# kcat/openal-soft

Measured on AMD Instinct MI355X. Metric: mixed voices/sec @48kHz 1024-sample update, HRTF stereo; fraction of HBM roofline, higher is better.
Workload: dtype f32

## Files before the change

### openal-soft_amd/csrc/api.hip

```cpp
#include "api_context.hpp"
namespace oalgpu {

thread_local std::string gLastError;

int Fail(int code, const std::string &msg)
{
    gLastError = msg;
    return code;
}

void ParkResidentContexts(int device);

int UseDevice(int device)
{
    int count = 0;
    if(hipGetDeviceCount(&count) != hipSuccess || count <= 0)
        return Fail(OALGPU_ERR_NO_DEVICE, "no HIP device available (the product has no CPU path)");
    if(device < 0 || device >= count) return Fail(OALGPU_ERR_INVALID, "device ordinal out of range");
    HIP_TRY(hipSetDevice(device));
    ParkResidentContexts(device);
    return OALGPU_OK;
}

}
// ... 493 lines not shown
        else (void)hipGetLastError();
    }
    return ResidentGiveUp(c, std::string(e < 4 ? what[e] : "a wait timed out") + state);
}

static int ResidentSubmit(oalgpu_context *c, uint32_t samples_to_do)
{
    auto &R = c->res;
    if(!R.ready) { if(int rc = ResidentInit(c)) return R.failed ? 1 : rc; }
    HIP_TRY(hipSetDevice(c->desc.device));
    using clk = std::chrono::steady_clock;
    std::unique_lock<std::mutex> g(gResLock);
    const DeviceLayout &L = c->L;
    const bool launchNow = !R.running;
    ResidentArgs a{};
    uint32_t evk = 0;
    bool timed = false;
    if(launchNow)
    {
        if(c->postPending) HIP_TRY(hipStreamWaitEvent(R.reduceStream, c->lastPostEvent ? c->lastPostEvent : c->evPostDone, 0));
        const uint32_t k = evk = R.launches % oalgpu_context::ResidentState::kEv;
        if(R.evOpen[k]) { HIP_TRY(hipEventSynchronize(R.evStop[k])); ResidentCollectTimes(c, false); }
        timed = R.timeLaunches;
        a.door = R.door; a.counters = R.counters.p; a.hostFlags = R.hostFlags; a.partBase = R.part.p; a.setStride = uint32_t(R.setFloats);
        a.base = R.next; a.endSeq = R.next + R.maxUpdates; a.redPerUpdate = R.redGroups;
        a.startedTarget = R.startedTotal + L.numGroups; a.launchId = R.launches + 1u;
        __atomic_store_n(&R.door->exitSeq[a.launchId & 3u], R.next + 0x40000000u, __ATOMIC_RELEASE);
        __atomic_store_n(&R.door->seq, R.next, __ATOMIC_RELEASE);
        __builtin_ia32_sfence();
    }
    {
        const auto deadline = clk::now() + std::chrono::seconds(5);
        uint32_t spins = 0;
        while(int32_t(R.posts - __atomic_load_n(R.hostFlags + 16u * kRhProgress, __ATOMIC_ACQUIRE)) >= int32_t(kResidentDepth))
        {
            __builtin_ia32_pause();
            if((++spins & 0x3ffu) == 0 && clk::now() > deadline)
            {
                ResidentParkLocked(c);
                g.unlock();
                (void)hipStreamSynchronize(c->stream); (void)hipStreamSynchronize(R.reduceStream); (void)hipStreamSynchronize(c->postStream);
                if(int rc = ResidentCheckError(c)) return rc;
                return ResidentGiveUp(c, "the post-process made no progress for 5 s");
            }
        }
    }
    if(__atomic_load_n(R.hostFlags + 16u * kRhError, __ATOMIC_RELAXED))
    {
        ResidentParkLocked(c);
        g.unlock();
        (void)hipStreamSynchronize(c->stream); (void)hipStreamSynchronize(R.reduceStream); (void)hipStreamSynchronize(c->postStream);
        return ResidentCheckError(c);
    }
    c->outRingWritten = false;
    oalgpu_param_block *b = R.pendingBlock;
    R.pendingBlock = nullptr;
    if(b) b->heldBy = nullptr;
    ResidentSlot &sl = R.door->slot[R.next % kResidentSlots];
    sl.recs = b ? reinterpret_cast<unsigned long long>(b->recs.p) : 0ull;
    sl.map = b ? reinterpret_cast<unsigned long long>(b->voiceToRec.p) : 0ull;
    sl.rows = b ? reinterpret_cast<unsigned long long>(b->rows.p) : 0ull;
    sl.samples = samples_to_do;
    __builtin_ia32_sfence();
    __atomic_store_n(&R.door->seq, R.next + 1u, __ATOMIC_RELEASE);
    __builtin_ia32_sfence();
    if(launchNow)
    {
        const uint32_t k = evk;
        HIP_TRY(LaunchVoiceWaveResident(c->stream, L, a, timed ? R.evStart[k] : nullptr, timed ? R.evStop[k] : nullptr));
        R.evOpen[k] = timed; R.evFirst[k] = R.next; R.evLast[k] = R.next;
        ++R.launches; R.startedTotal = a.startedTarget; R.endSeq = a.endSeq; R.launchBase = R.next;
        R.awaitStarted = a.launchId;
        R.running = true;
        gResRunning.push_back(c);
        gResCount.store(int(gResRunning.size()), std::memory_order_relaxed);
    }
    const uint32_t set = R.next % kResidentSets;
    if(R.awaitStarted)
    {
        const uint32_t id = R.awaitStarted;
        R.awaitStarted = 0u;
        const auto deadline = clk::now() + std::chrono::seconds(5);
        uint32_t spins = 0;
        while(__atomic_load_n(R.hostFlags + 16u * kRhResident, __ATOMIC_ACQUIRE) != id)
        {
            __builtin_ia32_pause();
            if((++spins & 0x3ffu) == 0 && clk::now() > deadline)
            {
                ++R.next;
                ResidentParkLocked(c);
                g.unlock();
                (void)hipStreamSynchronize(c->stream);
                return ResidentGiveUp(c, "its workgroups did not all start within 5 s");
            }
        }
    }
    if(R.copyPending) { HIP_TRY(hipStreamWaitEvent(R.reduceStream, R.copyPending, 0)); R.copyPending = nullptr; }
    DeviceLayout Lr = L;
    Lr.partHrtf = R.part.p + size_t{set} * R.setFloats;
    LaunchBusReduceResident(R.reduceStream, Lr, CarrySource(c, true), R.counters.p, R.hostFlags, set, (R.setUses[set] + 1u) * L.numGroups,
        R.posts * R.firGroups);
    HIP_TRY(hipGetLastError());
    ++R.setUses[set];
    c->lastPostEvent = c->evPostDone;
    if(int rc = PostDirectHrtfFused(c, c->postStream, samples_to_do, c->limOn ? nullptr : c->evPostDone, true)) return rc;
    if(c->limOn)
    {
        if(int rc = RunLimiter(c, c->postStream, samples_to_do)) return rc;
        HIP_TRY(hipEventRecord(c->evPostDone, c->postStream));
        R.copyPending = c->evPostDone;
    }
    c->postPending = true;
    ++R.next;
    ++c->updatesSubmitted;
    R.evLast[(R.launches - 1u) % oalgpu_context::ResidentState::kEv] = R.next;
    if(R.next == R.endSeq)
    {
// ... 403 lines not shown
```

### openal-soft_amd/csrc/kernels.hpp

```cpp
#pragma once
#include <hip/hip_runtime.h>
#include <stdint.h>

#include "dev_hrtf.hpp"
#include "dev_mix.hpp"
#include "dev_resample.hpp"
#include "dev_voice.hpp"
#include "../host/limiter_params.hpp"
#include "../host/uhj_params.hpp"
#include "../host/stabilizer_params.hpp"
#include "../host/crossfeed_params.hpp"

namespace oalgpu {

enum VoiceFlagBits : uint32_t {
    kFlagFading = 1u << 0,
    kFlagHasHrtf = 1u << 1,
    kFlagDirectFilter = 1u << 2,
    kFlagHrtfDirty = 1u << 3,
    kFlagAmbiScale = 1u << 4,
    kFlagNfc = 1u << 5,
    kFlagQueue = 1u << 7,
    kFlagDelayed = 1u << 6,
    kFlagSendFilterShift = 8
};

struct alignas(16) VoiceCtl {
    int32_t playState;
    int32_t position;
    uint32_t positionFrac;
    int32_t curBuffer;
    int32_t loopBuffer;
    uint32_t step;
    int32_t rsKind;
    uint32_t rsM, rsL;
    float rsSf;
    uint32_t rsFilterOffset;
    uint32_t flags;
    int32_t sendSlot[6];
    uint32_t hrtfOldDelay[2];
    float hrtfOldGain;
    uint32_t hrtfTgtDelay[2];
    float hrtfTgtGain;
    BufferItem buf;
};
static_assert(sizeof(VoiceCtl) == 128, "VoiceCtl is one 128-byte line");

struct alignas(16) AmbiScaleState { float coeff, lpZ1, lpZ2, apZ1, hfScale, lfScale; uint32_t pad[2]; };

struct alignas(16) NfcState { float a[5][5], b[5][5], z[5][4]; uint32_t pad[10]; };
static_assert(sizeof(NfcState) == 320, "NfcState");

struct alignas(16) BiquadSlot { BiquadState f; uint32_t pad[3]; };
static_assert(sizeof(BiquadSlot) == 64, "BiquadSlot");

__host__ __device__ inline uint32_t LineBlockDwords(uint32_t lineStride) { return 3u * lineStride + 8u; }

struct ParamRecord {
    uint32_t voice;
    uint32_t step;
// ... 62 lines not shown
    float pass, uint32_t lane)
{
    const uint32_t i0 = idx[0], i1 = idx[1], i2 = idx[2], i3 = idx[3];
    const float w0 = w[0], w1 = w[1], w2 = w[2], w3 = w[3];
    const uint32_t live = ((L.irSize + 1u) & ~1u) * 2u;
    for(uint32_t e = lane; e < L.irStride * 2; e += 64)
    {
        float x = (e < 2) ? pass : 0.0f;
        x = L.hrirs[size_t{i0} * (kHrirLen * 2) + e] * w0 + x;
        x = L.hrirs[size_t{i1} * (kHrirLen * 2) + e] * w1 + x;
        x = L.hrirs[size_t{i2} * (kHrirLen * 2) + e] * w2 + x;
        x = L.hrirs[size_t{i3} * (kHrirLen * 2) + e] * w3 + x;
        __builtin_nontemporal_store((e < live) ? x : 0.0f, &L.hrtfTgt[size_t{v} * L.irStride * 2 + e]);
    }
}

__device__ __forceinline__ void ApplyRecordWave(const DeviceLayout &L, const ParamRecord &r, uint32_t lane)
{
    const uint32_t v = r.voice;
    VoiceCtl &ctl = L.ctl[v];
    if(lane == 0)
    {
        ctl.step = r.step;
        ctl.rsKind = r.rsKind; ctl.rsM = r.rsM; ctl.rsL = r.rsL; ctl.rsSf = r.rsSf;
        ctl.rsFilterOffset = r.rsFilterOffset;
        const uint32_t keep = ctl.flags & (kFlagFading | kFlagHasHrtf | kFlagAmbiScale | kFlagNfc | kFlagDelayed | kFlagQueue
            | (r.keepHrtf ? uint32_t(kFlagHrtfDirty) : 0u));
        ctl.flags = keep | (r.flags & ~(kFlagFading | kFlagHasHrtf | kFlagHrtfDirty | kFlagAmbiScale | kFlagNfc | kFlagDelayed | kFlagQueue))
            | (L.hrtf ? (kFlagHasHrtf | (r.keepHrtf ? 0u : uint32_t(kFlagHrtfDirty))) : 0u);
        for(int i = 0; i < 6; ++i) ctl.sendSlot[i] = (uint32_t(i) < L.numSends) ? r.sendSlot[i] : -1;
        if(L.hrtf && !r.keepHrtf)
        {
            ctl.hrtfTgtDelay[0] = r.hrtfDelay[0]; ctl.hrtfTgtDelay[1] = r.hrtfDelay[1];
            ctl.hrtfTgtGain = r.hrtfGain;
        }
    }
    if(lane == 1) BiquadSetTarget(L.dfilt[size_t{v} * 2 + 0].f, r.dirLp);
    if(lane == 2) BiquadSetTarget(L.dfilt[size_t{v} * 2 + 1].f, r.dirHp);
    if(lane >= 8 && lane < 8 + 2 * L.numSends)
    {
        const uint32_t i = (lane - 8) >> 1, hp = (lane - 8) & 1u;
        BiquadSetTarget(L.sfilt[(size_t{v} * L.numSends + i) * 2 + hp].f, hp ? r.sendHp[i] : r.sendLp[i]);
    }
    if(L.hrtf) { if(!r.keepHrtf) ApplyHrtfTargetWave(L, v, r.hrtfIdx, r.hrtfW, r.hrtfPass, lane); }
    else if(lane < L.numDry)
        L.gainTgt[size_t{v} * L.numDry + lane] = r.dryGains[lane];
    for(uint32_t k = lane; k < L.numSends * L.wetChannels; k += 64)
        L.sendTgt[size_t{v} * L.numSends * L.wetChannels + k] = r.sendGains[k / L.wetChannels][k % L.wetChannels];
}

struct VoiceInitRecord { uint32_t voice; int32_t buffer, looping, position; uint32_t positionFrac; int32_t queue; };

constexpr uint32_t kResidentSets = 4;
constexpr uint32_t kResidentSlots = 16;
constexpr uint32_t kResidentDepth = 8;
constexpr unsigned long long kResidentWatchdogTicks = 200000000ull;

struct ResidentSlot { unsigned long long recs, map, rows; uint32_t samples, pad; };
struct alignas(64) ResidentDoor {
    uint32_t seq;
    uint32_t exitSeq[4];
    uint32_t pad[11];
    ResidentSlot slot[kResidentSlots];
};
enum ResidentCounter : uint32_t {
    kRcArrive0 = 0,
    kRcRedRead = 4,
    kRcRedDone = 5,
    kRcPostDone = 6,
    kRcStarted = 7,
    kRcWaitDoor = 8,
    kRcWaitRed = 9,
    kRcWaitArrive = 10,
    kRcWaitPost = 11,
    kRcWaitRedDone = 12,
    kRcWaitSplit = 13,
    kRcInstall = 14,
    kRcBusy = 15,
    kRcTop = 16,
    kRcCount = 17
};
enum ResidentHostFlag : uint32_t { kRhResident = 0, kRhError = 1, kRhProgress = 2,
    kRhFault = 3,
    kRhCount = 4 };
struct ResidentArgs {
    const ResidentDoor *door;
    uint32_t *counters;
    uint32_t *hostFlags;
    float *partBase;
    uint32_t setStride;
    uint32_t base, endSeq;
    uint32_t redPerUpdate;
    uint32_t startedTarget, launchId;
};

void LaunchResample(hipStream_t s, bool exact, const ResampleSpec &spec, const float *src, uint32_t frac,
    uint32_t increment, float *dst, uint32_t n);
void LaunchMix(hipStream_t s, const float *in, uint32_t n, float *out, uint32_t nlines, float *cur,
    const float *tgt, uint32_t counter, uint32_t outpos);
void LaunchMixHrtf(hipStream_t s, bool exact, const float *in, float *accum, uint32_t irsize, const float *coeffs,
    uint32_t dL, uint32_t dR, float gain, float step, const float *oldcoeffs, uint32_t odL, uint32_t odR,
    float oldgain, int blend, uint32_t n);
void LaunchMixDirectHrtf(hipStream_t s, bool exact, float *left, float *right, const float *in, uint32_t nch,
    float *accum, SplitterState *splitters, const float *hfscales, const float *chanCoeffs, uint32_t irsize,
    uint32_t n, float *temp);
void LaunchBiquadDual(hipStream_t s, BiquadState *f0, BiquadState *f1, const float *src, float *dst, uint32_t n);
void LaunchGetCoeffs(hipStream_t s, const HrtfStoreDev &st, const float *dirs, uint32_t count, float *coeffs,
    uint32_t *delays);

void LaunchPostDirectHrtfFast(hipStream_t s, float *left, float *right, const float *in, uint32_t nch, float *accum,
    SplitterState *splitters, const float *hfscales, const float *chanCoeffs, uint32_t irsize, uint32_t n, float *temp,
    hipEvent_t evDone = nullptr);

inline uint32_t ReducePostReduceGroups(const DeviceLayout &L) { return uint32_t((BusFloats(L) + 63u) / 64u); }
void LaunchReducePostFused(hipStream_t s, const DeviceLayout &L, const float *carry, float *left, float *right, const float *in, uint32_t nch,
    const float *accIn, float *carryOut, const SplitterState *spIn, SplitterState *spOut, const float *hfscales, const float *chanCoeffs,
    uint32_t irsize, uint32_t n, float *xf, uint32_t *arrived, uint32_t epoch, const float runPower[4], hipEvent_t evDone,
// ... 171 lines not shown
```

### openal-soft_amd/csrc/voice_wave.hip

```cpp
#include <hip/hip_ext.h>
#include "wave_common.hpp"

#pragma clang fp contract(off)

#ifndef OALGPU_WAVE_MIN_WG
#define OALGPU_WAVE_MIN_WG 2
#endif

namespace oalgpu {
namespace {
struct RowLineGain {
    float gain{0.0f}, cur{0.0f}, step{0.0f};
    uint32_t fadeLen{0};
    __device__ __forceinline__ void add(const MixLineGain &g)
    {
        const float constant = g.steady ? g.tgt : 0.0f;
        gain += constant;
        if(g.fadeLen) { cur += g.cur; step += g.step; fadeLen = g.fadeLen; }
        else cur += constant;
    }
};
__device__ __forceinline__ void StoreRowBlock(uint32_t *blk, uint32_t ls, uint32_t lane, const RowLineGain &r, bool live)
{
    uint32_t maxFade = r.fadeLen;
// ... 394 lines not shown
        {
            const uint32_t old = __hip_atomic_fetch_add(RA.counters + 16u * kRcStarted, 1u, __ATOMIC_RELAXED, __HIP_MEMORY_SCOPE_AGENT);
            if(old + 1u == RA.startedTarget)
                __hip_atomic_store(RA.hostFlags + 16u * kRhResident, RA.launchId, __ATOMIC_RELAXED, __HIP_MEMORY_SCOPE_SYSTEM);
        }
    }
    for(;;)
    {
    uint32_t tU = t, laneU = lane0;
    if constexpr (RES) asm volatile("" : "+v"(tU), "+v"(laneU));
    const uint32_t t = tU, lane0 = laneU;
    bool stageRows = true;
    if constexpr (RES)
    {
        const ResidentArgs &RA = next.res;
        if(t == 0)
        {
            const unsigned long long tTop = __builtin_amdgcn_s_memrealtime();
            uint32_t go = 0u, fault = 0u;
            unsigned long long recs = 0ull, map = 0ull, rowsP = 0ull;
            uint32_t smp = 0u;
            if(upd != RA.endSeq)
            {
                const ResidentDoor *door = RA.door;
                const uint32_t *exitp = &door->exitSeq[RA.launchId & 3u];
                const uint32_t *rr = RA.counters + 16u * kRcRedRead;
                const bool needRed = int32_t(upd - kResidentSets) >= 0;
                const uint32_t want = (upd - kResidentSets + 1u) * RA.redPerUpdate;
                unsigned long long t0 = 0ull;
                uint32_t waitedFor = 0u;
                for(uint32_t spins = 0;; ++spins)
                {
                    const uint32_t ex = ResLoadSys(exitp), sq = ResLoadSys(&door->seq), rd = needRed ? ResLoadDev(rr) : want;
                    if(int32_t(ex - upd) <= 0) break;
                    const bool rung = int32_t(sq - upd) > 0, redOk = int32_t(rd - want) >= 0;
                    if(rung && redOk) { go = 1u; break; }
                    if(spins == 0u) { t0 = __builtin_amdgcn_s_memrealtime(); waitedFor = rung ? 2u : 1u; }
                    else if((spins & 15u) == 15u && __builtin_amdgcn_s_memrealtime() - t0 > kResidentWatchdogTicks)
                    {
                        fault = 1u;
                        uint32_t *fi = RA.hostFlags + 16u * kRhFault;
                        fi[0] = upd; fi[1] = sq; fi[2] = ex; fi[3] = rd; fi[4] = want; fi[5] = group; fi[6] = RA.launchId;
                        fi[7] = uint32_t(__builtin_amdgcn_s_memrealtime() - t0);
                        break;
                    }
                    if(spins < 32u) __builtin_amdgcn_s_sleep(2); else __builtin_amdgcn_s_sleep(24);
                }
                if(waitedFor && (group & 127u) == 0u)
                    __hip_atomic_fetch_add(RA.counters + 16u * (waitedFor == 1u ? kRcWaitDoor : kRcWaitRed), uint32_t(__builtin_amdgcn_s_memrealtime() - t0),
                        __ATOMIC_RELAXED, __HIP_MEMORY_SCOPE_AGENT);
                if(go)
                {
                    const ResidentSlot *sl = &door->slot[upd % kResidentSlots];
                    recs = ResLoadSys(&sl->recs); map = ResLoadSys(&sl->map); rowsP = ResLoadSys(&sl->rows); smp = ResLoadSys(&sl->samples);
                }
            }
            if(fault) __hip_atomic_store(RA.hostFlags + 16u * kRhError, 1u, __ATOMIC_RELAXED, __HIP_MEMORY_SCOPE_SYSTEM);
            if((group & 127u) == 0u)
                __hip_atomic_fetch_add(RA.counters + 16u * kRcTop, uint32_t(__builtin_amdgcn_s_memrealtime() - tTop), __ATOMIC_RELAXED, __HIP_MEMORY_SCOPE_AGENT);
            sm.res[0] = go; sm.res[1] = smp;
            sm.res[2] = uint32_t(recs); sm.res[3] = uint32_t(recs >> 32); sm.res[4] = uint32_t(map); sm.res[5] = uint32_t(map >> 32);
            sm.res[8] = uint32_t(rowsP); sm.res[9] = uint32_t(rowsP >> 32);
        }
        __syncthreads();
        const unsigned long long tSeen = __builtin_amdgcn_s_memrealtime();
        if(__builtin_amdgcn_readfirstlane(sm.res[0]) == 0u) break;
        N = __builtin_amdgcn_readfirstlane(sm.res[1]);
        const unsigned long long recsU = (uint64_t{uint32_t(__builtin_amdgcn_readfirstlane(sm.res[3]))} << 32) | uint32_t(__builtin_amdgcn_readfirstlane(sm.res[2]));
        const unsigned long long mapU = (uint64_t{uint32_t(__builtin_amdgcn_readfirstlane(sm.res[5]))} << 32) | uint32_t(__builtin_amdgcn_readfirstlane(sm.res[4]));
        if(mapU)
        {
            const int32_t *map = reinterpret_cast<const int32_t*>(mapU);
            const ParamRecord *recs = reinterpret_cast<const ParamRecord*>(recsU);
            const unsigned long long rowsU = (uint64_t{uint32_t(__builtin_amdgcn_readfirstlane(sm.res[9]))} << 32) | uint32_t(__builtin_amdgcn_readfirstlane(sm.res[8]));
            const float *rows = reinterpret_cast<const float*>(rowsU);
            for(uint32_t j = 0; j < vCount; j += 2u)
                InstallPair(L, map, recs, rows, vBegin + 2u * j, vBegin + 2u * j + 2u, j + 1u < vCount, lane0);
        }
        asm volatile("s_waitcnt vmcnt(0) lgkmcnt(0)" ::: "memory");
        __syncthreads();
        __builtin_amdgcn_s_dcache_inv();
        asm volatile("s_waitcnt lgkmcnt(0)" ::: "memory");
        if(t == 0)
        {
            const unsigned long long tIn = __builtin_amdgcn_s_memrealtime();
            if((group & 127u) == 0u)
                __hip_atomic_fetch_add(RA.counters + 16u * kRcInstall, uint32_t(tIn - tSeen), __ATOMIC_RELAXED, __HIP_MEMORY_SCOPE_AGENT);
            sm.res[6] = uint32_t(tIn);
        }
    }
    VoiceHead headN{};
    VoiceTail tailN{};
    SrcPlan planN{false, 0u, 0u};
    BufferItem bufN{};
    bool loopingN = false;
    float fstC = 0.0f;
    const uint32_t keyVoice = group * kWWaves * vpw;
    const uint32_t lastVoice = L.numVoices - 1u;
    {
        const uint32_t v0 = vCount ? voiceAt(0) : lastVoice;
        headN = LoadHeadScalar(L.ctl + v0); bufN = LoadCtlBufferScalar(L.ctl + v0);
        if constexpr (NL == 0) tailN = LoadTailScalar(L.ctl + v0);
    }
    asm volatile("" ::: "memory");
    const VoiceHead headK = LoadHeadScalar(L.ctl + (keyVoice < L.numVoices ? keyVoice : lastVoice));
    asm volatile("" ::: "memory");
    const int psK = headK.playState, kK = headK.rsKind;
// ... 1011 lines not shown
```

### openal-soft_amd/csrc/voice_wave16.hip

```cpp
#define OALGPU_WAVE_NO_LAUNCHER
#include "voice_wave.hip"

#pragma clang fp contract(off)

namespace oalgpu {
namespace {

constexpr int kW16Outs = kLine / 64;

constexpr int kW16Rd = 1184;
constexpr int kW16Rd2 = kMaxEdge + kPre * 64 + 8;
constexpr int kW16Area = kResampleDataSize + kLine;
static_assert(kW16Rd % 64 == 32 && kW16Rd >= kMaxPad + kPre * 64 + 8, "rd2 sits half the banks away from rd");
static_assert(kW16Rd + kW16Rd2 <= kW16Area, "the twice-parked window fits");
static_assert(kResampleDataSize >= kLine + 64, "a send's filter scan parks the unfiltered samples in the window's area");
constexpr int kW16DumpF2 = 64 * 17 + 68;
static_assert(kW16DumpF2 * 2 <= kW16Area, "the dump fits");
struct W16PhaseB {
    uint32_t xh[2][kXhDw];
    uint32_t hr[2][kHrDw];
    uint32_t hro[2][kHrDw];
    float in0[2 * kHist];
};
static_assert(sizeof(W16PhaseB) <= size_t(kW16Area) * 4, "phase B fits the area (nothing of it is written before the sample line is back in registers)");
// ... 144 lines not shown
    for(uint32_t k = lane; k < uint32_t(2 * kHrDw); k += 64) hz32[k] = 0u;
    uint16_t *hz = reinterpret_cast<uint16_t*>(&hr[0][0]);
    const uint32_t u = 80u - lane;
    hz[0 * kHrHalves + u] = uint16_t(hi); hz[1 * kHrHalves + u] = uint16_t(lo);
    return __builtin_bit_cast(float, __builtin_amdgcn_readfirstlane(__builtin_bit_cast(int, inv)));
}

__device__ __forceinline__ uint32_t W16VoiceOf(uint32_t group, uint32_t wave, uint32_t waves)
{
    const uint32_t a = wave >> 2, b = wave & 3u;
    return group * waves + 4u * a + ((a + b) & 3u);
}

struct Next16 { const ParamRecord *recs; const int32_t *map; const float *rows; ResidentArgs res; };
struct W16Sends {
    BiquadSlot *sfilt; const float *sendTgt; float *sendCur; float *streams; uint32_t *lineGains;
    uint32_t numSends, wetCh, lineStride, spv;
};

template<bool PROF, int WAVES, bool SENDS = false, bool RES = false>
__global__ void OALGPU_SINGLE_DS_OPS __launch_bounds__(WAVES * 64) VoiceWave16Kernel(WaveArgsHrtf L, uint32_t samplesToDo, Next16 next, WaveProf prof, W16Sends S)
{
    unsigned long long tEntry = 0;
    if constexpr (PROF) tEntry = __builtin_readcyclecounter();
    constexpr uint32_t kW16Waves = uint32_t(WAVES), kW16Threads = uint32_t(WAVES) * 64u;
    __shared__ W16Wg<WAVES> sm;
    const uint32_t t = threadIdx.x;
    uint32_t lane = t & 63u;
    const uint32_t wave = __builtin_amdgcn_readfirstlane(t >> 6);
    const uint32_t group = blockIdx.x;
    const uint32_t irStride = L.irStride;
    uint32_t N = samplesToDo;
    W16Lds &w = sm.w[wave];
    asm volatile("; argument block resident" :: "s"(L.tables), "s"(L.buffers), "s"(L.ctl), "s"(L.prev), "s"(L.dfilt), "s"(L.hrtfOld),
        "s"(L.hrtfTgt), "s"(L.hist), "s"(L.ambi), "s"(L.startDelay), "s"(L.queueDone), "s"(L.partHrtf), "s"(L.hrirs),
        "s"(next.recs), "s"(next.map), "s"(L.numVoices), "s"(L.irStride), "s"(L.pad), "s"(samplesToDo));

    const uint32_t vRaw = W16VoiceOf(group, wave, kW16Waves);
    const bool haveVoice = vRaw < L.numVoices;
    const uint32_t lastVoice = L.numVoices - 1u;
    const uint32_t v = haveVoice ? vRaw : lastVoice;
    const uint32_t keyVoice = group * uint32_t(kW16Waves);

    uint32_t upd = 0u, updBase = 0u;
    if constexpr (RES)
    {
        const ResidentArgs &RA = next.res;
        upd = updBase = RA.base;
        if(t == 0)
        {
            const uint32_t old = __hip_atomic_fetch_add(RA.counters + 16u * kRcStarted, 1u, __ATOMIC_RELAXED, __HIP_MEMORY_SCOPE_AGENT);
            if(old + 1u == RA.startedTarget)
                __hip_atomic_store(RA.hostFlags + 16u * kRhResident, RA.launchId, __ATOMIC_RELAXED, __HIP_MEMORY_SCOPE_SYSTEM);
        }
    }
    for(;;)
    {
    uint32_t tU = threadIdx.x;
    if constexpr (RES) { asm volatile("" : "+v"(tU)); lane = tU & 63u; }
    const uint32_t t = tU;
    if constexpr (RES)
    {
        const ResidentArgs &RA = next.res;
        if(t == 0)
        {
            const unsigned long long tTop = __builtin_amdgcn_s_memrealtime();
            uint32_t go = 0u, fault = 0u;
            unsigned long long recs = 0ull, map = 0ull, rowsP = 0ull;
            uint32_t smp = 0u;
            if(upd != RA.endSeq)
            {
                const ResidentDoor *door = RA.door;
                const uint32_t *exitp = &door->exitSeq[RA.launchId & 3u];
                const uint32_t *rr = RA.counters + 16u * kRcRedRead;
                const bool needRed = int32_t(upd - kResidentSets) >= 0;
                const uint32_t want = (upd - kResidentSets + 1u) * RA.redPerUpdate;
                unsigned long long t0 = 0ull;
                uint32_t waitedFor = 0u;
                for(uint32_t spins = 0;; ++spins)
                {
                    const uint32_t ex = ResLoadSys(exitp), sq = ResLoadSys(&door->seq), rd = needRed ? ResLoadDev(rr) : want;
                    if(int32_t(ex - upd) <= 0) break;
                    const bool rung = int32_t(sq - upd) > 0, redOk = int32_t(rd - want) >= 0;
                    if(rung && redOk) { go = 1u; break; }
                    if(spins == 0u) { t0 = __builtin_amdgcn_s_memrealtime(); waitedFor = rung ? 2u : 1u; }
                    else if((spins & 15u) == 15u && __builtin_amdgcn_s_memrealtime() - t0 > kResidentWatchdogTicks)
                    {
                        fault = 1u;
                        uint32_t *fi = RA.hostFlags + 16u * kRhFault;
                        fi[0] = upd; fi[1] = sq; fi[2] = ex; fi[3] = rd; fi[4] = want; fi[5] = group; fi[6] = RA.launchId;
                        fi[7] = uint32_t(__builtin_amdgcn_s_memrealtime() - t0);
                        break;
                    }
                    if(spins < 32u) __builtin_amdgcn_s_sleep(2); else __builtin_amdgcn_s_sleep(24);
                }
                if(waitedFor && (group & 127u) == 0u)
                    __hip_atomic_fetch_add(RA.counters + 16u * (waitedFor == 1u ? kRcWaitDoor : kRcWaitRed), uint32_t(__builtin_amdgcn_s_memrealtime() - t0),
                        __ATOMIC_RELAXED, __HIP_MEMORY_SCOPE_AGENT);
                if(go)
                {
                    const ResidentSlot *sl = &door->slot[upd % kResidentSlots];
                    recs = ResLoadSys(&sl->recs); map = ResLoadSys(&sl->map); rowsP = ResLoadSys(&sl->rows); smp = ResLoadSys(&sl->samples);
                }
            }
            if(fault) __hip_atomic_store(RA.hostFlags + 16u * kRhError, 1u, __ATOMIC_RELAXED, __HIP_MEMORY_SCOPE_SYSTEM);
            if((group & 127u) == 0u)
                __hip_atomic_fetch_add(RA.counters + 16u * kRcTop, uint32_t(__builtin_amdgcn_s_memrealtime() - tTop), __ATOMIC_RELAXED, __HIP_MEMORY_SCOPE_AGENT);
            sm.res[0] = go; sm.res[1] = smp;
            sm.res[2] = uint32_t(recs); sm.res[3] = uint32_t(recs >> 32); sm.res[4] = uint32_t(map); sm.res[5] = uint32_t(map >> 32);
            sm.res[8] = uint32_t(rowsP); sm.res[9] = uint32_t(rowsP >> 32);
        }
        __syncthreads();
        const unsigned long long tSeen = __builtin_amdgcn_s_memrealtime();
        if(__builtin_amdgcn_readfirstlane(sm.res[0]) == 0u) break;
        N = __builtin_amdgcn_readfirstlane(sm.res[1]);
        const unsigned long long recsU = (uint64_t{uint32_t(__builtin_amdgcn_readfirstlane(sm.res[3]))} << 32) | uint32_t(__builtin_amdgcn_readfirstlane(sm.res[2]));
        const unsigned long long mapU = (uint64_t{uint32_t(__builtin_amdgcn_readfirstlane(sm.res[5]))} << 32) | uint32_t(__builtin_amdgcn_readfirstlane(sm.res[4]));
        if(mapU && haveVoice)
        {
            const unsigned long long rowsU = (uint64_t{uint32_t(__builtin_amdgcn_readfirstlane(sm.res[9]))} << 32) | uint32_t(__builtin_amdgcn_readfirstlane(sm.res[8]));
            InstallPair(L, reinterpret_cast<const int32_t*>(mapU), reinterpret_cast<const ParamRecord*>(recsU), reinterpret_cast<const float*>(rowsU), v, v, false, lane);
        }
        asm volatile("s_waitcnt vmcnt(0) lgkmcnt(0)" ::: "memory");
        __syncthreads();
        __builtin_amdgcn_s_dcache_inv();
        asm volatile("s_waitcnt lgkmcnt(0)" ::: "memory");
        if(t == 0)
        {
            const unsigned long long tIn = __builtin_amdgcn_s_memrealtime();
            if((group & 127u) == 0u)
                __hip_atomic_fetch_add(RA.counters + 16u * kRcInstall, uint32_t(tIn - tSeen), __ATOMIC_RELAXED, __HIP_MEMORY_SCOPE_AGENT);
            sm.res[6] = uint32_t(tIn);
        }
    }
    auto stamp = [&](int slot)
    {
        if constexpr (PROF) { if(prof.times && haveVoice && (t & 63u) == 0u) prof.times[size_t{v} * 8 + slot] = __builtin_readcyclecounter(); }
    };
    if constexpr (PROF) { if(prof.times && haveVoice && (t & 63u) == 0u) prof.times[size_t{v} * 8 + 0] = tEntry; }
    auto stamp2 = [&](int slot)
    {
        if constexpr (PROF) { if(prof.times && haveVoice && (t & 63u) == 0u) prof.times[size_t{L.numVoices} * 8 + size_t{v} * 8 + slot] = __builtin_readcyclecounter(); }
    };
    const VoiceHead head = LoadHeadScalar(L.ctl + v);
    const BufferItem buf = LoadCtlBufferScalar(L.ctl + v);
    const VoiceTail tail = LoadTailScalar(L.ctl + v);
    asm volatile("" ::: "memory");
    const VoiceHead headK = LoadHeadScalar(L.ctl + (keyVoice < L.numVoices ? keyVoice : lastVoice));
    asm volatile("" ::: "memory");
    const int psK = headK.playState, kK = headK.rsKind;
    const uint32_t mK = kK == 2 ? 4u : headK.rsM, lK = kK == 2 ? 1u : headK.rsL, offK = headK.rsFilterOffset;

    const bool eligK = keyVoice < L.numVoices && (kK == 2 || (kK == 3 && (mK == 12 || mK == 24)))
        && (psK == OALGPU_VOICE_PLAYING || psK == OALGPU_VOICE_STOPPING);
    bool stageRows = true;
    if constexpr (RES) { if(upd != updBase) stageRows = !(eligK && sm.tabKey == offK * 8u + uint32_t(kK) && sm.tabM == mK); }
    if constexpr (RES) __syncthreads();
// ... 524 lines not shown
                    c.playState = OALGPU_VOICE_STOPPING;
                }
            }
        }
    }

    if(!RES && next.map && haveVoice)
    {
        __builtin_amdgcn_fence(__ATOMIC_RELEASE, "workgroup");
        if(next.rows && irStride <= 64u) InstallPair(L, next.map, next.recs, next.rows, v, v, false, lane);
        else
        {
            const int32_t ri = __builtin_amdgcn_readfirstlane(next.map[v]);
            if(ri >= 0) ApplyNextRecord(L, next.recs[ri], lane);
        }
    }
    stamp(5);
    {
        WaveSync();
        f2 *dump = w.dump;
        const uint32_t jc = lane & 15u, q4 = lane >> 4;
#pragma unroll
        for(int T = 0; T < 4; ++T)
#pragma unroll
            for(int r = 0; r < 4; ++r)
                dump[17u * (16u * uint32_t(T) + jc) + 4u * q4 + uint32_t(r)] = f2{accM[0][T][r], accM[1][T][r]};
        if(jc < 4u)
        {
#pragma unroll
            for(int r = 0; r < 4; ++r) dump[17u * (64u + jc) + 4u * q4 + uint32_t(r)] = f2{accM[0][4][r], accM[1][4][r]};
        }
        __syncthreads();
        f2 *ph = reinterpret_cast<f2*>(L.partHrtf) + size_t{group} * (kLine + kHrirLen);
        if constexpr (RES)
            ph = reinterpret_cast<f2*>(next.res.partBase + size_t{upd % kResidentSets} * next.res.setStride) + size_t{group} * (kLine + kHrirLen);
        for(uint32_t k = t; k < uint32_t(kLine + kHrirLen); k += uint32_t(kW16Threads))
        {
            f2 s = {0.0f, 0.0f};
            if(k < 64u * 17u)
            {
                const uint32_t at = k + (k >> 4);
                s = sm.w[0].dump[at];
#pragma unroll
                for(int ww = 1; ww < WAVES; ++ww) { const f2 o = sm.w[ww].dump[at]; s.x += o.x; s.y += o.y; }
            }
            if constexpr (RES) StorePartialCoherent(&ph[k], s);
            else StorePartial(&ph[k], s);
        }
    }
    stamp(6);
    if constexpr (!RES) break;
    else
    {
        asm volatile("s_waitcnt vmcnt(0)" ::: "memory");
        __syncthreads();
        if(t == 0)
        {
            __hip_atomic_fetch_add(next.res.counters + 16u * (kRcArrive0 + upd % kResidentSets), 1u, __ATOMIC_RELAXED, __HIP_MEMORY_SCOPE_AGENT);
            if((group & 127u) == 0u)
                __hip_atomic_fetch_add(next.res.counters + 16u * kRcBusy, uint32_t(__builtin_amdgcn_s_memrealtime()) - sm.res[6], __ATOMIC_RELAXED, __HIP_MEMORY_SCOPE_AGENT);
        }
        ++upd;
    }
    }
}

}

bool Wave16Applies(const DeviceLayout &L)
{
    if(!(L.hrtf && L.firMfma && L.irStride >= 8 && L.irStride <= 64 && L.sliceLines == 0 && L.nfc == nullptr)) return false;
    if(L.numSends == 0) return L.accLines == 0;
    return L.numSends <= 6 && L.mixLines >= 1 && L.mixLines <= 32 && L.wetChannels <= 32u;
}
uint32_t Wave16WavesFor(uint32_t voices, uint32_t cus)
{
    for(uint32_t w : {4u, 8u}) if((voices + w - 1u) / w <= cus) return w;
    return 16u;
}
uint32_t Wave16Groups(const DeviceLayout &L) { return (L.numVoices + L.wave16 - 1u) / L.wave16; }
const char *Wave16KernelName(const DeviceLayout &L)
{
    if(L.numSends) return L.wave16 == 16u ? "VoiceWave16Kernel<16, sends>" : (L.wave16 == 8u ? "VoiceWave16Kernel<8, sends>" : "VoiceWave16Kernel<4, sends>");
    return L.wave16 == 16u ? "VoiceWave16Kernel<16>" : (L.wave16 == 8u ? "VoiceWave16Kernel<8>" : "VoiceWave16Kernel<4>");
}

hipError_t LaunchVoiceWave16(hipStream_t s, const DeviceLayout &L, uint32_t samplesToDo, const WaveProf *prof, hipEvent_t evStart, hipEvent_t evStop,
    const ParamRecord *nextRecs, const int32_t *nextMap, const float *nextRows)
{
    const Next16 next{nextRecs, nextMap, nextRows, ResidentArgs{}};
    const WaveProf none{nullptr, 0u};
    const dim3 grid(Wave16Groups(L)), block(L.wave16 * 64u);
    const W16Sends S{L.sfilt, L.sendTgt, L.sendCur, L.streams, L.lineGains, L.numSends, L.wetChannels, L.lineStride, L.streamsPerVoice};
#define OALGPU_W16_LAUNCH(P, W, SD, PA) hipExtLaunchKernelGGL((VoiceWave16Kernel<P, W, SD>), grid, block, 0, s, evStart, evStop, 0u, WaveArgsHrtf{L}, samplesToDo, next, PA, S)
    if(L.numSends)
    {
        const Next16 noNext{nullptr, nullptr, nullptr, ResidentArgs{}};
        if(L.wave16 == 16u) hipExtLaunchKernelGGL((VoiceWave16Kernel<false, 16, true>), grid, block, 0, s, evStart, nullptr, 0u, WaveArgsHrtf{L}, samplesToDo, noNext, none, S);
        else if(L.wave16 == 8u) hipExtLaunchKernelGGL((VoiceWave16Kernel<false, 8, true>), grid, block, 0, s, evStart, nullptr, 0u, WaveArgsHrtf{L}, samplesToDo, noNext, none, S);
        else hipExtLaunchKernelGGL((VoiceWave16Kernel<false, 4, true>), grid, block, 0, s, evStart, nullptr, 0u, WaveArgsHrtf{L}, samplesToDo, noNext, none, S);
        if(hipError_t e = hipGetLastError(); e != hipSuccess) return e;
        return LaunchStreamRowsMix(s, L, samplesToDo, L.wave16, evStop);
    }
    if(prof)
    {
        if(L.wave16 == 16u) OALGPU_W16_LAUNCH(true, 16, false, *prof); else if(L.wave16 == 8u) OALGPU_W16_LAUNCH(true, 8, false, *prof); else OALGPU_W16_LAUNCH(true, 4, false, *prof);
    }
    else
    {
        if(L.wave16 == 16u) OALGPU_W16_LAUNCH(false, 16, false, none); else if(L.wave16 == 8u) OALGPU_W16_LAUNCH(false, 8, false, none); else OALGPU_W16_LAUNCH(false, 4, false, none);
    }
#undef OALGPU_W16_LAUNCH
    return hipGetLastError();
}
// ... 17 lines not shown
```

Before: 115.4 million.

## Tag doorbell slots with sequence to poll one slot and drop end-of-update barrier

The doorbell slot now carries a 16-bit update tag in the upper bits of each 48-bit pointer plus a sequence/samples word. The resident kernel polls the slot directly instead of polling seq and then re-reading the slot, which saves a round trip over system memory. The end-of-update workgroup barrier is replaced by a per-wave shared-memory arrival count, so the last wave to arrive signals the reduce stage. This adds a host check that pointers fit in 48 bits and relies on tag consistency across separate 64-bit stores.

After: 111.1 million. -3.7%, worse.

```diff
diff --git a/openal-soft_amd/csrc/api.hip b/openal-soft_amd/csrc/api.hip
--- a/openal-soft_amd/csrc/api.hip
+++ b/openal-soft_amd/csrc/api.hip
@@ -569,17 +569,27 @@
         (void)hipStreamSynchronize(c->stream); (void)hipStreamSynchronize(R.reduceStream); (void)hipStreamSynchronize(c->postStream);
         return ResidentCheckError(c);
     }
+    if(oalgpu_param_block *pb = R.pendingBlock)
+    {
+        const ResidentUpdate px{reinterpret_cast<unsigned long long>(pb->recs.p), reinterpret_cast<unsigned long long>(pb->voiceToRec.p),
+            reinterpret_cast<unsigned long long>(pb->rows.p), 0u};
+        if(!ResidentPointersFit(px))
+        {
+            ResidentParkLocked(c);
+            g.unlock();
+            return ResidentGiveUp(c, "a parameter block lies above the 48-bit addresses a doorbell slot holds");
+        }
+    }
     c->outRingWritten = false;
     oalgpu_param_block *b = R.pendingBlock;
     R.pendingBlock = nullptr;
     if(b) b->heldBy = nullptr;
-    ResidentSlot &sl = R.door->slot[R.next % kResidentSlots];
-    sl.recs = b ? reinterpret_cast<unsigned long long>(b->recs.p) : 0ull;
-    sl.map = b ? reinterpret_cast<unsigned long long>(b->voiceToRec.p) : 0ull;
-    sl.rows = b ? reinterpret_cast<unsigned long long>(b->rows.p) : 0ull;
-    sl.samples = samples_to_do;
-    __builtin_ia32_sfence();
-    __atomic_store_n(&R.door->seq, R.next + 1u, __ATOMIC_RELEASE);
+    ResidentUpdate x{};
+    x.recs = b ? reinterpret_cast<unsigned long long>(b->recs.p) : 0ull;
+    x.map = b ? reinterpret_cast<unsigned long long>(b->voiceToRec.p) : 0ull;
+    x.rows = b ? reinterpret_cast<unsigned long long>(b->rows.p) : 0ull;
+    x.samples = samples_to_do;
+    ResidentPublish(R.door, R.next, x);
     __builtin_ia32_sfence();
     if(launchNow)
     {
diff --git a/openal-soft_amd/csrc/kernels.hpp b/openal-soft_amd/csrc/kernels.hpp
--- a/openal-soft_amd/csrc/kernels.hpp
+++ b/openal-soft_amd/csrc/kernels.hpp
@@ -6,6 +6,7 @@
 #include "dev_mix.hpp"
 #include "dev_resample.hpp"
 #include "dev_voice.hpp"
+#include "resident_door.hpp"
 #include "../host/limiter_params.hpp"
 #include "../host/uhj_params.hpp"
 #include "../host/stabilizer_params.hpp"
@@ -174,17 +175,7 @@
 struct VoiceInitRecord { uint32_t voice; int32_t buffer, looping, position; uint32_t positionFrac; int32_t queue; };
 
 constexpr uint32_t kResidentSets = 4;
-constexpr uint32_t kResidentSlots = 16;
-constexpr uint32_t kResidentDepth = 8;
 constexpr unsigned long long kResidentWatchdogTicks = 200000000ull;
-
-struct ResidentSlot { unsigned long long recs, map, rows; uint32_t samples, pad; };
-struct alignas(64) ResidentDoor {
-    uint32_t seq;
-    uint32_t exitSeq[4];
-    uint32_t pad[11];
-    ResidentSlot slot[kResidentSlots];
-};
 enum ResidentCounter : uint32_t {
     kRcArrive0 = 0,
     kRcRedRead = 4,
diff --git a/openal-soft_amd/csrc/resident_door.hpp b/openal-soft_amd/csrc/resident_door.hpp
--- /dev/null
+++ b/openal-soft_amd/csrc/resident_door.hpp
@@ -0,0 +1,46 @@
+#pragma once
+#include <stdint.h>
+
+namespace oalgpu {
+
+constexpr uint32_t kResidentSlots = 16;
+constexpr uint32_t kResidentDepth = 8;
+
+struct alignas(32) ResidentSlot { unsigned long long recs, map, rows, last; };
+constexpr unsigned long long kResidentPtrMask = (1ull << 48) - 1ull;
+struct ResidentUpdate { unsigned long long recs, map, rows; uint32_t samples; };
+
+struct alignas(64) ResidentDoor {
+    uint32_t seq;
+    uint32_t exitSeq[4];
+    uint32_t pad[11];
+    ResidentSlot slot[kResidentSlots];
+};
+
+inline bool ResidentPointersFit(const ResidentUpdate &x) { return ((x.recs | x.map | x.rows) & ~kResidentPtrMask) == 0ull; }
+
+inline void ResidentPublish(ResidentDoor *door, uint32_t u, const ResidentUpdate &x)
+{
+    const unsigned long long tag = static_cast<unsigned long long>((u + 1u) & 0xffffu) << 48;
+    ResidentSlot &sl = door->slot[u % kResidentSlots];
+    __atomic_store_n(&sl.recs, x.recs | tag, __ATOMIC_RELAXED);
+    __atomic_store_n(&sl.map, x.map | tag, __ATOMIC_RELAXED);
+    __atomic_store_n(&sl.rows, x.rows | tag, __ATOMIC_RELAXED);
+    __atomic_store_n(&sl.last, (static_cast<unsigned long long>(u + 1u) << 32) | x.samples, __ATOMIC_RELEASE);
+#if defined(__x86_64__)
+    __builtin_ia32_sfence();
+#endif
+    __atomic_store_n(&door->seq, u + 1u, __ATOMIC_RELEASE);
+}
+
+#if defined(__HIPCC__)
+__host__ __device__
+#endif
+inline bool ResidentSlotIs(uint32_t u, unsigned long long recs, unsigned long long map, unsigned long long rows, unsigned long long last, ResidentUpdate &x)
+{
+    const unsigned long long tag = (u + 1u) & 0xffffu;
+    x.recs = recs & kResidentPtrMask; x.map = map & kResidentPtrMask; x.rows = rows & kResidentPtrMask; x.samples = static_cast<uint32_t>(last);
+    return static_cast<uint32_t>(last >> 32) == u + 1u && (recs >> 48) == tag && (map >> 48) == tag && (rows >> 48) == tag;
+}
+
+}
diff --git a/openal-soft_amd/csrc/voice_wave.hip b/openal-soft_amd/csrc/voice_wave.hip
--- a/openal-soft_amd/csrc/voice_wave.hip
+++ b/openal-soft_amd/csrc/voice_wave.hip
@@ -470,7 +470,9 @@
                 if(go)
                 {
                     const ResidentSlot *sl = &door->slot[upd % kResidentSlots];
-                    recs = ResLoadSys(&sl->recs); map = ResLoadSys(&sl->map); rowsP = ResLoadSys(&sl->rows); smp = ResLoadSys(&sl->samples);
+                    ResidentUpdate x;
+                    (void)ResidentSlotIs(upd, ResLoadSys(&sl->recs), ResLoadSys(&sl->map), ResLoadSys(&sl->rows), ResLoadSys(&sl->last), x);
+                    recs = x.recs; map = x.map; rowsP = x.rows; smp = x.samples;
                 }
             }
             if(fault) __hip_atomic_store(RA.hostFlags + 16u * kRhError, 1u, __ATOMIC_RELAXED, __HIP_MEMORY_SCOPE_SYSTEM);
diff --git a/openal-soft_amd/csrc/voice_wave16.hip b/openal-soft_amd/csrc/voice_wave16.hip
--- a/openal-soft_amd/csrc/voice_wave16.hip
+++ b/openal-soft_amd/csrc/voice_wave16.hip
@@ -220,8 +220,20 @@
             const uint32_t old = __hip_atomic_fetch_add(RA.counters + 16u * kRcStarted, 1u, __ATOMIC_RELAXED, __HIP_MEMORY_SCOPE_AGENT);
             if(old + 1u == RA.startedTarget)
                 __hip_atomic_store(RA.hostFlags + 16u * kRhResident, RA.launchId, __ATOMIC_RELAXED, __HIP_MEMORY_SCOPE_SYSTEM);
-        }
-    }
+            sm.res[7] = 0u;
+        }
+    }
+    [[maybe_unused]] auto countIn = [&](uint32_t u)
+    {
+        asm volatile("s_waitcnt vmcnt(0)" ::: "memory");
+        const uint32_t n = __hip_atomic_fetch_add(&sm.res[7], 1u, __ATOMIC_RELAXED, __HIP_MEMORY_SCOPE_WORKGROUP) + 1u;
+        if(n % uint32_t(WAVES) == 0u)
+        {
+            __hip_atomic_fetch_add(next.res.counters + 16u * (kRcArrive0 + u % kResidentSets), 1u, __ATOMIC_RELAXED, __HIP_MEMORY_SCOPE_AGENT);
+            if((group & 127u) == 0u)
+                __hip_atomic_fetch_add(next.res.counters + 16u * kRcBusy, uint32_t(__builtin_amdgcn_s_memrealtime()) - sm.res[6], __ATOMIC_RELAXED, __HIP_MEMORY_SCOPE_AGENT);
+        }
+    };
     for(;;)
     {
     uint32_t tU = threadIdx.x;
@@ -241,22 +253,26 @@
                 const ResidentDoor *door = RA.door;
                 const uint32_t *exitp = &door->exitSeq[RA.launchId & 3u];
                 const uint32_t *rr = RA.counters + 16u * kRcRedRead;
+                const ResidentSlot *sl = &door->slot[upd % kResidentSlots];
                 const bool needRed = int32_t(upd - kResidentSets) >= 0;
                 const uint32_t want = (upd - kResidentSets + 1u) * RA.redPerUpdate;
                 unsigned long long t0 = 0ull;
                 uint32_t waitedFor = 0u;
                 for(uint32_t spins = 0;; ++spins)
                 {
-                    const uint32_t ex = ResLoadSys(exitp), sq = ResLoadSys(&door->seq), rd = needRed ? ResLoadDev(rr) : want;
+                    const uint32_t ex = ResLoadSys(exitp), rd = needRed ? ResLoadDev(rr) : want;
+                    const unsigned long long w0 = ResLoadSys(&sl->recs), w1 = ResLoadSys(&sl->map), w2 = ResLoadSys(&sl->rows), w3 = ResLoadSys(&sl->last);
+                    if(spins == 0u && upd != updBase) countIn(upd - 1u);
                     if(int32_t(ex - upd) <= 0) break;
-                    const bool rung = int32_t(sq - upd) > 0, redOk = int32_t(rd - want) >= 0;
-                    if(rung && redOk) { go = 1u; break; }
+                    ResidentUpdate x;
+                    const bool rung = ResidentSlotIs(upd, w0, w1, w2, w3, x), redOk = int32_t(rd - want) >= 0;
+                    if(rung && redOk) { go = 1u; recs = x.recs; map = x.map; rowsP = x.rows; smp = x.samples; break; }
                     if(spins == 0u) { t0 = __builtin_amdgcn_s_memrealtime(); waitedFor = rung ? 2u : 1u; }
                     else if((spins & 15u) == 15u && __builtin_amdgcn_s_memrealtime() - t0 > kResidentWatchdogTicks)
                     {
                         fault = 1u;
                         uint32_t *fi = RA.hostFlags + 16u * kRhFault;
-                        fi[0] = upd; fi[1] = sq; fi[2] = ex; fi[3] = rd; fi[4] = want; fi[5] = group; fi[6] = RA.launchId;
+                        fi[0] = upd; fi[1] = uint32_t(w3 >> 32); fi[2] = ex; fi[3] = rd; fi[4] = want; fi[5] = group; fi[6] = RA.launchId;
                         fi[7] = uint32_t(__builtin_amdgcn_s_memrealtime() - t0);
                         break;
                     }
@@ -265,12 +281,8 @@
                 if(waitedFor && (group & 127u) == 0u)
                     __hip_atomic_fetch_add(RA.counters + 16u * (waitedFor == 1u ? kRcWaitDoor : kRcWaitRed), uint32_t(__builtin_amdgcn_s_memrealtime() - t0),
                         __ATOMIC_RELAXED, __HIP_MEMORY_SCOPE_AGENT);
-                if(go)
-                {
-                    const ResidentSlot *sl = &door->slot[upd % kResidentSlots];
-                    recs = ResLoadSys(&sl->recs); map = ResLoadSys(&sl->map); rowsP = ResLoadSys(&sl->rows); smp = ResLoadSys(&sl->samples);
-                }
-            }
+            }
+            else if(upd != updBase) countIn(upd - 1u);
             if(fault) __hip_atomic_store(RA.hostFlags + 16u * kRhError, 1u, __ATOMIC_RELAXED, __HIP_MEMORY_SCOPE_SYSTEM);
             if((group & 127u) == 0u)
                 __hip_atomic_fetch_add(RA.counters + 16u * kRcTop, uint32_t(__builtin_amdgcn_s_memrealtime() - tTop), __ATOMIC_RELAXED, __HIP_MEMORY_SCOPE_AGENT);
@@ -901,14 +913,7 @@
     if constexpr (!RES) break;
     else
     {
-        asm volatile("s_waitcnt vmcnt(0)" ::: "memory");
-        __syncthreads();
-        if(t == 0)
-        {
-            __hip_atomic_fetch_add(next.res.counters + 16u * (kRcArrive0 + upd % kResidentSets), 1u, __ATOMIC_RELAXED, __HIP_MEMORY_SCOPE_AGENT);
-            if((group & 127u) == 0u)
-                __hip_atomic_fetch_add(next.res.counters + 16u * kRcBusy, uint32_t(__builtin_amdgcn_s_memrealtime()) - sm.res[6], __ATOMIC_RELAXED, __HIP_MEMORY_SCOPE_AGENT);
-        }
+        if(wave != 0u && lane == 0u) countIn(upd);
         ++upd;
     }
     }
```
